# bghira/SimpleTuner

Hardware: NVIDIA H100
Metric: images/sec Flux.1-dev LoRA bf16 1024^2 (higher is better)
Workload: dtype bf16

## Files before the change

### simpletuner_b200/csrc/api.cu

```cuda
#include <cuda.h>
#include <cudaTypedefs.h>
#include <cuda_runtime.h>

#include <algorithm>
#include <atomic>
#include <cstdarg>
#include <cstdio>
#include <cmath>
#include <cstdlib>
#include <cstring>
#include <mutex>
#include <string>
#include <unordered_map>

#include <climits>
#include "../../include/stb200.h"
#include "attn_bwd.cuh"
#include "attn_fwd.cuh"
#include "optim.cuh"
#include "elementwise.cuh"
#include "gemm.cuh"
#include "lokr.cuh"
#include "vae.cuh"
#include "wgrad.cuh"
// ... 176 lines not shown
    cfg.attrs = attr;
    cfg.numAttrs = 1;
    static std::atomic<int> max_clusters{0};
    int mc = max_clusters.load(std::memory_order_acquire);
    if (mc == 0) {
      cfg.gridDim = dim3(CLUSTER * (num_sms() / CLUSTER));
      STB_CUDA(cudaOccupancyMaxActiveClusters(&mc, kernel, &cfg));
      if (mc < 1) return fail(STB_ERR_CUDA, "%s: no %d-CTA cluster of this kernel fits on the device", name, CLUSTER);
      max_clusters.store(mc, std::memory_order_release);
    }
    cfg.gridDim = dim3((unsigned)(CLUSTER * std::min<long long>(units, mc)));
    STB_CUDA(cudaLaunchKernelEx(&cfg, kernel, maps, p));
  }
  STB_LAUNCH_CHECK(name);
  return 0;
}

template <int BN>
int launch_gemm(const stb_gemm_args* a, cudaStream_t st, bool cluster) {
  stb::GemmMaps maps;
  std::memset(&maps, 0, sizeof maps);
  stb::GemmParams p;
  std::memset(&p, 0, sizeof p);
  for (int s = 0; s < a->nseg; ++s) {
    const stb_gemm_seg& g = a->seg[s];
    if (g.K <= 0 || (g.K & 7)) return fail(STB_ERR_ARG, "segment %d: K=%d must be a positive multiple of 8", s, g.K);
    if (int r = make_token_map(&maps.a[s], g.a, g.K, a->rows_per_batch, a->num_batches, g.a_row_stride, g.a_batch_stride,
                               stb::GemmCfg<BN>::BM))
      return r;
    if (g.w_kn) {
      unsigned long long wd[2] = {(unsigned long long)a->N, (unsigned long long)g.K};
      unsigned long long ws[1] = {(unsigned long long)g.w_row_stride * 2ull};
      unsigned wb[2] = {64, 64};
      if (int r = make_map(&maps.w[s], g.w, 2, wd, ws, wb)) return r;
    } else {
      unsigned long long wd[2] = {(unsigned long long)g.K, (unsigned long long)a->N};
      unsigned long long ws[1] = {(unsigned long long)g.w_row_stride * 2ull};
      unsigned wb[2] = {64, cluster ? 64u : (unsigned)BN};
      if (int r = make_map(&maps.w[s], g.w, 2, wd, ws, wb)) return r;
    }
    p.w_kn[s] = g.w_kn ? 1 : 0;
    p.kblocks[s] = (g.K + 63) / 64;
  }
  p.rows_per_batch = a->rows_per_batch;
  p.num_batches = a->num_batches;
  p.N = a->N;
  p.nseg = a->nseg;
  p.nan_to_num = a->nan_to_num;
  p.D = static_cast<__nv_bfloat16*>(a->d);
  p.d_batch_stride = a->d_batch_stride;
  p.d_row_stride = a->d_row_stride;
  p.bias = static_cast<const __nv_bfloat16*>(a->bias);
  p.gate = static_cast<const __nv_bfloat16*>(a->gate);
  p.gate_batch_stride = a->gate_batch_stride;
  p.res = static_cast<const __nv_bfloat16*>(a->res);
  p.res_batch_stride = a->res_batch_stride;
  p.res_row_stride = a->res_row_stride;
  p.aux = static_cast<__nv_bfloat16*>(a->aux);
  p.aux_batch_stride = a->aux_batch_stride;
  p.aux_row_stride = a->aux_row_stride;
  auto go = [&](auto epi) -> int {
    constexpr int EPI = decltype(epi)::value;
    if constexpr (BN == 128)
      if (cluster) return launch_gemm_kernel<BN, EPI, false, 2>(maps, p, st, "gemm_bf16_tn_cluster");
    return launch_gemm_kernel<BN, EPI, false>(maps, p, st, "gemm_bf16_tn");
  };
  switch (a->epi) {
    case stb::EPI_STORE: return go(std::integral_constant<int, stb::EPI_STORE>{});
    case stb::EPI_GELU: return go(std::integral_constant<int, stb::EPI_GELU>{});
    case stb::EPI_GATE_RES: return go(std::integral_constant<int, stb::EPI_GATE_RES>{});
    case stb::EPI_MUL_DGELU: return go(std::integral_constant<int, stb::EPI_MUL_DGELU>{});
    case stb::EPI_ADD_RES: return go(std::integral_constant<int, stb::EPI_ADD_RES>{});
    case stb::EPI_MUL: return go(std::integral_constant<int, stb::EPI_MUL>{});
    case stb::EPI_QUICK_GELU: return go(std::integral_constant<int, stb::EPI_QUICK_GELU>{});
  }
  return fail(STB_ERR_ARG, "unknown epilogue %d", a->epi);
}

bool aligned16(const void* p) { return (reinterpret_cast<uintptr_t>(p) & 15) == 0; }

}

template <int HD, bool BIAS, bool KEY = false>
static int launch_attn_fwd(const stb::AttnFwdMaps& maps, const stb::AttnFwdParams& p, dim3 grid, cudaStream_t st) {
  using Cfg = stb::AttnFwdCfg<HD>;
  constexpr int SMEM = Cfg::SMEM_BYTES + (KEY ? Cfg::KV_STAGES * 128 * 4 : 0);
  if (int r = set_smem<stb::attn_fwd_kernel<HD, BIAS, KEY>>(SMEM)) return r;
  stb::attn_fwd_kernel<HD, BIAS, KEY><<<grid, 384, SMEM, st>>>(maps, p);
  STB_LAUNCH_CHECK(KEY ? "attn_fwd_key_bias" : (BIAS ? "attn_fwd_bias" : "attn_fwd"));
  return 0;
}

template <int HD, bool BIAS>
static int launch_attn_bwd(const stb_attn_bwd_args* a, const stb::AttnBwdMaps& maps, const stb::AttnBwdParams& p,
                           cudaStream_t st) {
  {
    const long long warps = (long long)a->B * a->Sq * a->H;
    stb::attn_bwd_delta_kernel<HD><<<(unsigned)((warps + 7) / 8), 256, 0, st>>>(
        static_cast<const __nv_bfloat16*>(a->o), a->o_b, a->o_s, a->o_h,
        static_cast<const __nv_bfloat16*>(a->d_o), a->do_b, a->do_s, a->do_h, a->delta, a->B, a->H, a->Sq);
    STB_LAUNCH_CHECK("attn_bwd_delta");
  }
  using Cfg = stb::AttnBwdCfg<HD>;
  constexpr int SMEM1 = Cfg::DKDV_SMEM_BYTES, SMEM2 = Cfg::DQ_SMEM_BYTES + (BIAS ? Cfg::STAGES * Cfg::KB : 0);
  if (int r = set_smem<stb::attn_bwd_dkdv_kernel<HD, BIAS>>(SMEM1)) return r;
  if (int r = set_smem<stb::attn_bwd_dq_kernel<HD, BIAS>>(SMEM2)) return r;
  stb::attn_bwd_dkdv_kernel<HD, BIAS><<<dim3((a->Sk + 63) / 64, a->H, a->B), 384, SMEM1, st>>>(maps, p);
  STB_LAUNCH_CHECK(BIAS ? "attn_bwd_dkdv_bias" : "attn_bwd_dkdv");
  stb::attn_bwd_dq_kernel<HD, BIAS><<<dim3((a->Sq + 127) / 128, a->H, a->B), 384, SMEM2, st>>>(maps, p);
  STB_LAUNCH_CHECK(BIAS ? "attn_bwd_dq_bias" : "attn_bwd_dq");
  return 0;
}

template <int BN, int OUT>
static int launch_wgrad(const stb::WgradMaps& maps, stb::WgradParams p, cudaStream_t st) {
  constexpr int SMEM = stb::WgradCfg<BN, OUT>::SMEM_BYTES;
  if (int r = set_smem<stb::wgrad_kernel<BN, OUT>>(SMEM)) return r;
  p.col_tiles = (p.K + BN - 1) / BN;
  const int units = p.splits * ((p.N + 127) / 128) * p.col_tiles;
  const int grid = OUT == stb::WGRAD_OUT_BF16_NK ? std::min(units, num_sms()) : units;
  stb::wgrad_kernel<BN, OUT><<<grid, 384, SMEM, st>>>(maps, p);
  STB_LAUNCH_CHECK(OUT == stb::WGRAD_OUT_BF16_NK ? "wgrad_full" : "wgrad_tn");
  return 0;
}

extern "C" {

const char* stb_last_error(void) { return g_err.c_str(); }
int stb_version(void) { return 100; }
long long stb_launch_count(void) { return g_launches.load(); }
void stb_reset_launch_count(void) { g_launches.store(0); }

int stb_gemm_bf16(const stb_gemm_args* a, void* stream) {
  if (int r = check_device()) return r;
  if (!a || a->nseg < 1 || a->nseg > 3) return fail(STB_ERR_ARG, "nseg must be 1..3");
  if (a->num_batches < 1 || a->rows_per_batch < 1 || a->N < 1) return fail(STB_ERR_ARG, "empty problem");
  if (!aligned16(a->d) || (a->d_row_stride & 7) || (a->d_batch_stride & 7))
    return fail(STB_ERR_ARG, "D must be 16-byte aligned with strides multiple of 8 elements");
  if (a->bias && !aligned16(a->bias)) return fail(STB_ERR_ARG, "bias must be 16-byte aligned");
  if (a->epi == STB_EPI_GATE_RES && (!a->gate || !a->res)) return fail(STB_ERR_ARG, "GATE_RES needs gate and res");
  if (a->epi == STB_EPI_GATE_RES && (!aligned16(a->gate) || (a->gate_batch_stride & 7)))
    return fail(STB_ERR_ARG, "gate must be 16-byte aligned");
  if ((a->epi == STB_EPI_GATE_RES || a->epi == STB_EPI_ADD_RES) &&
      (!a->res || !aligned16(a->res) || (a->res_row_stride & 7) || (a->res_batch_stride & 7)))
    return fail(STB_ERR_ARG, "res must be given, 16-byte aligned, strides multiple of 8");
  if ((a->epi == STB_EPI_MUL_DGELU || a->epi == STB_EPI_MUL) && !a->aux) return fail(STB_ERR_ARG, "MUL_DGELU / MUL need aux");
  if (a->aux && (!aligned16(a->aux) || (a->aux_row_stride & 7) || (a->aux_batch_stride & 7)))
    return fail(STB_ERR_ARG, "aux must be 16-byte aligned, strides multiple of 8");
  if (a->epi < 0 || a->epi > 6) return fail(STB_ERR_ARG, "unknown epilogue %d", a->epi);
  cudaStream_t st = static_cast<cudaStream_t>(stream);
  if (a->tile_mt < 0 || a->tile_mt > 2) return fail(STB_ERR_ARG, "unsupported tile config MT=%d", a->tile_mt);
  int bn = a->tile_bn;
  if (bn == 0) {
    bn = a->N <= 64 ? 64 : (a->rows_per_batch <= 64 && a->N > 128 ? 256 : 128);
  }
  if (bn == 256) return launch_gemm<256>(a, st, false);
  if (bn == 128) {
    const long long tiles_m = (long long)((a->rows_per_batch + 127) / 128) * a->num_batches;
    const bool cluster = a->tile_mt == 2 || (a->tile_mt == 0 && tiles_m >= 16 &&
                                             (a->epi == STB_EPI_GELU || a->epi == STB_EPI_MUL_DGELU));
    return launch_gemm<128>(a, st, cluster);
  }
  if (bn == 64) return launch_gemm<64>(a, st, false);
  return fail(STB_ERR_ARG, "unsupported tile config BN=%d", bn);
}

int stb_attn_fwd(const stb_attn_fwd_args* a, void* stream) {
  if (int r = check_device()) return r;
  if (!a || a->B < 1 || a->H < 1 || a->Sq < 1 || a->Sk < 1) return fail(STB_ERR_ARG, "empty attention problem");
  if (a->HD != 128 && a->HD != 64) return fail(STB_ERR_UNSUPPORTED, "head_dim %d not supported (64 or 128)", a->HD);
  if (!aligned16(a->o) || (a->o_s & 7) || (a->o_h & 7) || (a->o_b & 7)) return fail(STB_ERR_ARG, "O alignment");
  cudaStream_t st = static_cast<cudaStream_t>(stream);
  stb::AttnFwdMaps maps;
  auto mk = [&](CUtensorMap* m, const void* ptr, long long sb, long long ss, long long sh, int S) {
    return make_head_map(m, ptr, a->HD, a->H, S, a->B, sb, ss, sh, 128);
  };
  if (int r = mk(&maps.q, a->q, a->q_b, a->q_s, a->q_h, a->Sq)) return r;
  if (int r = mk(&maps.k, a->k, a->k_b, a->k_s, a->k_h, a->Sk)) return r;
  if (int r = mk(&maps.v, a->v, a->v_b, a->v_s, a->v_h, a->Sk)) return r;
  stb::AttnFwdParams p;
  p.B = a->B; p.H = a->H; p.Sq = a->Sq; p.Sk = a->Sk;
  p.scale = a->scale;
  p.O = static_cast<__nv_bfloat16*>(a->o);
  p.o_b = a->o_b; p.o_s = a->o_s; p.o_h = a->o_h;
  p.lse = a->lse;
  p.bias = static_cast<const __nv_bfloat16*>(a->bias);
  p.bias_b = a->bias_b; p.bias_h = a->bias_h; p.bias_q = a->bias_q;
  p.inv_scale = a->scale != 0.f ? 1.f / a->scale : 0.f;
  const dim3 grid((a->Sq + 127) / 128, a->H, a->B);
  if (a->bias) {
    const bool key_row = a->bias_q == 0 && a->bias_h == 0;
    if (a->scale == 0.f || a->bias_b < 0 || a->bias_h < 0 || (a->bias_q < a->Sk && !key_row))
      return fail(STB_ERR_ARG, "attn_fwd bias: scale must be non-zero, strides non-negative, and bias_q >= Sk "
                               "(or bias_q = bias_h = 0 for a per-key row)");
    if (key_row)
      return a->HD == 128 ? launch_attn_fwd<128, true, true>(maps, p, grid, st) : launch_attn_fwd<64, true, true>(maps, p, grid, st);
    return a->HD == 128 ? launch_attn_fwd<128, true>(maps, p, grid, st) : launch_attn_fwd<64, true>(maps, p, grid, st);
  }
  return a->HD == 128 ? launch_attn_fwd<128, false>(maps, p, grid, st) : launch_attn_fwd<64, false>(maps, p, grid, st);
}

int stb_attn_bwd(const stb_attn_bwd_args* a, void* stream) {
  if (int r = check_device()) return r;
  if (!a || a->B < 1 || a->H < 1 || a->Sq < 1 || a->Sk < 1) return fail(STB_ERR_ARG, "empty attention problem");
  if (a->HD != 128 && a->HD != 64) return fail(STB_ERR_UNSUPPORTED, "head_dim %d not supported (64 or 128)", a->HD);
  if (!a->lse || !a->delta) return fail(STB_ERR_ARG, "attn_bwd needs lse and a delta scratch buffer");
  auto al = [&](const void* ptr, long long sb, long long ss, long long sh) {
    return aligned16(ptr) && !(sb & 7) && !(ss & 7) && !(sh & 7);
  };
  if (!al(a->dq, a->dq_b, a->dq_s, a->dq_h) || !al(a->dk, a->dk_b, a->dk_s, a->dk_h) ||
      !al(a->dv, a->dv_b, a->dv_s, a->dv_h))
    return fail(STB_ERR_ARG, "dq/dk/dv must be 16-byte aligned with strides multiple of 8 elements");
  cudaStream_t st = static_cast<cudaStream_t>(stream);
  stb::AttnBwdMaps maps;
  auto mk = [&](CUtensorMap* m, const void* ptr, long long sb, long long ss, long long sh, int S, unsigned rows) {
    return make_head_map(m, ptr, a->HD, a->H, S, a->B, sb, ss, sh, rows);
  };
  if (int r = mk(&maps.q128, a->q, a->q_b, a->q_s, a->q_h, a->Sq, 128)) return r;
  if (int r = mk(&maps.do128, a->d_o, a->do_b, a->do_s, a->do_h, a->Sq, 128)) return r;
  if (int r = mk(&maps.q64, a->q, a->q_b, a->q_s, a->q_h, a->Sq, 64)) return r;
  if (int r = mk(&maps.k64, a->k, a->k_b, a->k_s, a->k_h, a->Sk, 64)) return r;
  if (int r = mk(&maps.v64, a->v, a->v_b, a->v_s, a->v_h, a->Sk, 64)) return r;
  if (int r = mk(&maps.do64, a->d_o, a->do_b, a->do_s, a->do_h, a->Sq, 64)) return r;
  stb::AttnBwdParams p;
  p.B = a->B; p.H = a->H; p.Sq = a->Sq; p.Sk = a->Sk;
  p.scale = a->scale;
  p.lse = a->lse;
  p.delta = a->delta;
  p.dq = static_cast<__nv_bfloat16*>(a->dq);
  p.dk = static_cast<__nv_bfloat16*>(a->dk);
  p.dv = static_cast<__nv_bfloat16*>(a->dv);
  p.dq_b = a->dq_b; p.dq_s = a->dq_s; p.dq_h = a->dq_h;
  p.dk_b = a->dk_b; p.dk_s = a->dk_s; p.dk_h = a->dk_h;
  p.dv_b = a->dv_b; p.dv_s = a->dv_s; p.dv_h = a->dv_h;
  p.fuse_prep = 0;
  if (const stb_qk_prep* f = a->qk_prep) {
    if (a->Sq != a->Sk) return fail(STB_ERR_ARG, "qk_prep fusion needs self-attention (Sq == Sk)");
    if (!f->src || !aligned16(f->src) || (f->src_b & 7) || (f->src_s & 7) || (f->k_off & 7))
      return fail(STB_ERR_ARG, "qk_prep.src must be 16-byte aligned with strides / k_off multiple of 8 elements");
    if ((f->cos_t == nullptr) != (f->sin_t == nullptr)) return fail(STB_ERR_ARG, "qk_prep: give both cos_t and sin_t or neither");
    p.fuse_prep = 1;
    p.src = static_cast<const __nv_bfloat16*>(f->src);
    p.src_b = f->src_b; p.src_s = f->src_s; p.k_off = f->k_off;
    p.wq0 = static_cast<const __nv_bfloat16*>(f->wq); p.wk0 = static_cast<const __nv_bfloat16*>(f->wk);
    p.wq1 = static_cast<const __nv_bfloat16*>(f->wq_added); p.wk1 = static_cast<const __nv_bfloat16*>(f->wk_added);
    p.s_split = f->s_split;
    p.cosT = f->cos_t; p.sinT = f->sin_t;
    p.eps = f->eps;
  }
  p.q = static_cast<const __nv_bfloat16*>(a->q);
  p.d_o = static_cast<const __nv_bfloat16*>(a->d_o);
  p.q_b = a->q_b; p.q_s = a->q_s; p.q_h = a->q_h;
  p.do_b = a->do_b; p.do_s = a->do_s; p.do_h = a->do_h;
  p.bias = static_cast<const __nv_bfloat16*>(a->bias);
  p.bias_b = a->bias_b;
  if (a->bias) {
    if (a->bias_b < 0 || (a->bias_b != 0 && a->bias_b < a->Sk))
      return fail(STB_ERR_UNSUPPORTED, "attn_bwd bias: only a per-key bias [B or 1, Sk] (bias_b = 0 or >= Sk) is supported");
    return a->HD == 128 ? launch_attn_bwd<128, true>(a, maps, p, st) : launch_attn_bwd<64, true>(a, maps, p, st);
  }
  return a->HD == 128 ? launch_attn_bwd<128, false>(a, maps, p, st) : launch_attn_bwd<64, false>(a, maps, p, st);
}

int stb_ln_modulate_fwd(const void* x, long long x_b, long long x_s, const void* shift, const void* scale,
                        long long mod_b, void* out, long long o_b, long long o_s, int B, int S, int D,
                        float eps, void* stream) {
  if (int r = check_device()) return r;
  if ((D & 7) || D > 8192) return fail(STB_ERR_ARG, "D=%d must be a multiple of 8 and <= 8192", D);
  if (!aligned16(x) || !aligned16(out) || !aligned16(shift) || !aligned16(scale) || (x_s & 7) || (x_b & 7) ||
      (o_s & 7) || (o_b & 7) || (mod_b & 7))
    return fail(STB_ERR_ARG, "ln_modulate_fwd alignment");
  cudaStream_t st = static_cast<cudaStream_t>(stream);
  const int rows = B * S;
  const int vpt = (D + 1023) / 1024;
  auto X = static_cast<const __nv_bfloat16*>(x);
  auto SH = static_cast<const __nv_bfloat16*>(shift);
  auto SC = static_cast<const __nv_bfloat16*>(scale);
  auto O = static_cast<__nv_bfloat16*>(out);
#define STB_LN_F(V) stb::ln_modulate_fwd_kernel<V><<<rows, 128, 0, st>>>(X, x_b, x_s, SH, SC, mod_b, O, o_b, o_s, S, D, eps)
  switch (vpt) {
    case 1: STB_LN_F(1); break;
    case 2: STB_LN_F(2); break;
// ... 562 lines not shown
```

### simpletuner_b200/csrc/attn_bwd.cuh

```cuda
#pragma once
#include "../../include/stb200.h"
#include "attn_fwd.cuh"
#include "common.cuh"
#include "elementwise.cuh"

namespace stb {

struct AttnBwdParams {
  int B, H, Sq, Sk;
  float scale;
  const float* lse;
  const float* delta;
  __nv_bfloat16 *dq, *dk, *dv;
  long long dq_b, dq_s, dq_h, dk_b, dk_s, dk_h, dv_b, dv_s, dv_h;
  const __nv_bfloat16 *q, *d_o;
  long long q_b, q_s, q_h, do_b, do_s, do_h;
  int fuse_prep;
  const __nv_bfloat16* src;
  long long src_b, src_s;
  int k_off;
  const __nv_bfloat16 *wq0, *wk0, *wq1, *wk1;
  int s_split;
  const float *cosT, *sinT;
  float eps;
  const __nv_bfloat16* bias;
  long long bias_b;
};

struct AttnBwdMaps {
  CUtensorMap q128, do128, q64, k64, v64, do64;
};

template <int HD>
__global__ void __launch_bounds__(256)
attn_bwd_delta_kernel(const __nv_bfloat16* __restrict__ o, long long o_b, long long o_s, long long o_h,
                      const __nv_bfloat16* __restrict__ d_o, long long do_b, long long do_s, long long do_h,
                      float* __restrict__ delta, int B, int H, int S) {
  constexpr int EPL = HD / 32;
  const long long wid = (long long)blockIdx.x * 8 + (threadIdx.x >> 5);
  if (wid >= (long long)B * S * H) return;
  const int lane = threadIdx.x & 31;
  const int h = int(wid % H);
  const long long r = wid / H;
  const int s = int(r % S);
  const int b = int(r / S);
  const __nv_bfloat16* po = o + b * o_b + s * o_s + h * o_h + lane * EPL;
  const __nv_bfloat16* pg = d_o + b * do_b + s * do_s + h * do_h + lane * EPL;
  float acc = 0.f;
#pragma unroll
  for (int i = 0; i < EPL; ++i) acc += __bfloat162float(po[i]) * __bfloat162float(pg[i]);
#pragma unroll
  for (int off = 16; off > 0; off >>= 1) acc += __shfl_xor_sync(0xffffffffu, acc, off);
  if (lane == 0) delta[((long long)b * H + h) * S + s] = acc;
}

template <int HD>
struct AttnBwdCfg {
  static constexpr int BIG = 128 * HD * 2;
  static constexpr int SMALL = 64 * HD * 2;
  static constexpr int STAGES = 3;
  static constexpr int STAT = 64 * 8;
  static constexpr int PT = 64 * 64 * 4;
  static constexpr int DKDV_SMEM_BYTES = 2 * SMALL + STAGES * (2 * SMALL + STAT) + 2 * PT + 1024 + 256;
  static constexpr int DQ_SMEM_BYTES = 2 * BIG + STAGES * 2 * SMALL + 1024 + 256;
  static constexpr int KB = 64 * 4;
};

__device__ __forceinline__ void named_bar_sync(int id, int nthreads) {
  asm volatile("bar.sync %0, %1;" ::"r"(id), "r"(nthreads) : "memory");
}
__device__ __forceinline__ void named_bar_arrive(int id, int nthreads) {
  asm volatile("bar.arrive %0, %1;" ::"r"(id), "r"(nthreads) : "memory");
}

template <int HD>
__device__ __forceinline__ void stage_acc(float* rows, const float (&acc)[HD / 2], float mul) {
  const int t = threadIdx.x & 127, wq = t >> 5, lane = t & 31;
#pragma unroll
  for (int i = 0; i < HD / 8; ++i)
#pragma unroll
    for (int hh = 0; hh < 2; ++hh) {
      float* r = rows + (wq * 16 + (lane >> 2) + 8 * hh) * (HD + 4) + 8 * i + 2 * (lane & 3);
      r[0] = acc[4 * i + 2 * hh] * mul;
      r[1] = acc[4 * i + 2 * hh + 1] * mul;
    }
}

template <int HD>
__device__ __forceinline__ void store_row_half(const float* row, int half, __nv_bfloat16* grow, bool row_ok, bool prep,
                                               const __nv_bfloat16* xrow, const __nv_bfloat16* w, const float* cs,
                                               const float* sn, float eps) {
  constexpr int NC = HD / 2;
  const int c0 = half * NC;
  if (!prep) {
    if (row_ok) {
#pragma unroll
      for (int c = 0; c < NC; c += 8) {
        float o[8];
#pragma unroll
        for (int i = 0; i < 8; ++i) o[i] = row[c0 + c + i];
        *reinterpret_cast<uint4*>(grow + c0 + c) = pack8(o);
      }
    }
    return;
  }
  float ss = 0.f, sgx = 0.f;
  float g[NC];
#pragma unroll
  for (int c = 0; c < NC; c += 8) {
    float x[8], wv[8];
    unpack8(row_ok ? __ldg(reinterpret_cast<const uint4*>(xrow + c0 + c)) : make_uint4(0u, 0u, 0u, 0u), x);
    if (w) unpack8(__ldg(reinterpret_cast<const uint4*>(w + c0 + c)), wv);
#pragma unroll
    for (int i = 0; i < 8; i += 2) {
      const int j = c0 + c + i;
      const float go0 = row[j], go1 = row[j + 1];
      float dy0 = go0, dy1 = go1;
      if (cs && row_ok) {
        const float2 c2 = __ldg(reinterpret_cast<const float2*>(cs + j));
        const float2 s2 = __ldg(reinterpret_cast<const float2*>(sn + j));
        dy0 = go0 * c2.x + go1 * s2.y;
        dy1 = go1 * c2.y - go0 * s2.x;
      }
      const float g0 = w ? dy0 * wv[i] : dy0, g1 = w ? dy1 * wv[i + 1] : dy1;
      ss += x[i] * x[i] + x[i + 1] * x[i + 1];
      sgx += g0 * x[i] + g1 * x[i + 1];
      g[c + i] = g0;
      g[c + i + 1] = g1;
    }
  }
  ss += __shfl_xor_sync(0xffffffffu, ss, 1);
  sgx += __shfl_xor_sync(0xffffffffu, sgx, 1);
  const float rstd = rsqrtf(ss / HD + eps);
  const float m = sgx * rstd / HD;
  if (row_ok) {
#pragma unroll
    for (int c = 0; c < NC; c += 8) {
      float x[8], o[8];
      unpack8(__ldg(reinterpret_cast<const uint4*>(xrow + c0 + c)), x);
#pragma unroll
      for (int i = 0; i < 8; ++i) o[i] = rstd * (g[c + i] - (x[i] * rstd) * m);
      *reinterpret_cast<uint4*>(grow + c0 + c) = pack8(o);
    }
  }
}

__device__ __forceinline__ void wgmma_ss_n64_zero(float (&d)[32], uint64_t a, uint64_t b) {
  asm volatile(
      "{\n\t.reg .pred p;\n\tsetp.ne.b32 p, %34, 0;\n\t"
      "wgmma.mma_async.sync.aligned.m64n64k16.f32.bf16.bf16 {%0, %1, %2, %3, %4, %5, %6, %7, %8, %9, %10, %11, %12, %13, "
      "%14, %15, %16, %17, %18, %19, %20, %21, %22, %23, %24, %25, %26, %27, %28, %29, %30, %31}, %32, %33, p, 1, 1, 0, 0;\n\t}\n"
      : "=f"(d[0]), "=f"(d[1]), "=f"(d[2]), "=f"(d[3]), "=f"(d[4]), "=f"(d[5]), "=f"(d[6]), "=f"(d[7]), "=f"(d[8]),
        "=f"(d[9]), "=f"(d[10]), "=f"(d[11]), "=f"(d[12]), "=f"(d[13]), "=f"(d[14]), "=f"(d[15]), "=f"(d[16]),
        "=f"(d[17]), "=f"(d[18]), "=f"(d[19]), "=f"(d[20]), "=f"(d[21]), "=f"(d[22]), "=f"(d[23]), "=f"(d[24]),
        "=f"(d[25]), "=f"(d[26]), "=f"(d[27]), "=f"(d[28]), "=f"(d[29]), "=f"(d[30]), "=f"(d[31])
      : "l"(a), "l"(b), "r"(0u));
// ... 359 lines not shown
```

### simpletuner_b200/csrc/attn_fwd.cuh

```cuda
#pragma once
#include "common.cuh"

namespace stb {

struct AttnFwdParams {
  int B, H, Sq, Sk;
  float scale;
  __nv_bfloat16* O;
  long long o_b, o_s, o_h;
  float* lse;
  const __nv_bfloat16* bias;
  long long bias_h, bias_q;
  float inv_scale;
  long long bias_b;
};

struct AttnFwdMaps {
  CUtensorMap q, k, v;
};

template <int HD>
struct AttnFwdCfg {
  static constexpr int ATOMS = HD / 64;
  static constexpr int TILE_BYTES = 128 * HD * 2;
  static constexpr int KV_STAGES = 2;
  static constexpr int SMEM_BYTES = TILE_BYTES + KV_STAGES * 2 * TILE_BYTES + 1024 + 256;
  static constexpr int THREADS = 384;
};

template <int R>
__device__ __forceinline__ void acc_to_afrag(const float (&d)[R], int kk, uint32_t (&a)[4]) {
  a[0] = pack_bf16x2(d[8 * kk + 0], d[8 * kk + 1]);
  a[1] = pack_bf16x2(d[8 * kk + 2], d[8 * kk + 3]);
  a[2] = pack_bf16x2(d[8 * kk + 4], d[8 * kk + 5]);
  a[3] = pack_bf16x2(d[8 * kk + 6], d[8 * kk + 7]);
}

template <int N>
__device__ __forceinline__ void wgmma_rs_mn(float (&d)[N / 2], const uint32_t (&a)[4], uint64_t b, uint32_t accumulate) {
  if constexpr (N == 128) wgmma_rs_n128<1>(d, a, b, accumulate);
  else wgmma_rs_n64<1>(d, a, b, accumulate);
}

template <int HD, bool BIAS = false, bool KEY = false>
__global__ void __launch_bounds__(384, 1)
attn_fwd_kernel(const __grid_constant__ AttnFwdMaps maps, const AttnFwdParams p) {
  using Cfg = AttnFwdCfg<HD>;
  constexpr int ATOMS = Cfg::ATOMS;
  constexpr int TILE = Cfg::TILE_BYTES;
  constexpr int ATOM_BYTES = 128 * 64 * 2;
  constexpr int NSTG = Cfg::KV_STAGES;

  extern __shared__ uint8_t smem_raw[];
  const uint32_t smem_base = (smem_u32(smem_raw) + 1023u) & ~1023u;
  const uint32_t q_smem = smem_base;
  const uint32_t k_smem = q_smem + TILE;
  const uint32_t v_smem = k_smem + NSTG * TILE;
  const uint32_t bar_base = v_smem + NSTG * TILE;
  const uint32_t q_full = bar_base;
  auto k_full = [&](int s) { return bar_base + 8u * (1 + s); };
  auto k_empty = [&](int s) { return bar_base + 8u * (1 + NSTG + s); };
  auto v_full = [&](int s) { return bar_base + 8u * (1 + 2 * NSTG + s); };
  auto v_empty = [&](int s) { return bar_base + 8u * (1 + 3 * NSTG + s); };
  auto b_full = [&](int s) { return bar_base + 8u * (1 + 4 * NSTG + s); };
  auto b_empty = [&](int s) { return bar_base + 8u * (1 + 5 * NSTG + s); };
  float* kb_rows = reinterpret_cast<float*>(smem_raw + (bar_base + 256 - smem_u32(smem_raw)));

  const int warp = threadIdx.x >> 5;
  const int lane = threadIdx.x & 31;
  const int wg = __shfl_sync(0xffffffffu, warp >> 2, 0);
  const int q0 = blockIdx.x * 128;
  const int h = blockIdx.y;
  const int b = blockIdx.z;
  const int n_kv = (p.Sk + 127) / 128;

  if (threadIdx.x == 0) {
    tma_prefetch_desc(&maps.q);
    tma_prefetch_desc(&maps.k);
    tma_prefetch_desc(&maps.v);
    mbar_init(q_full, 1);
    for (int s = 0; s < NSTG; ++s) {
      mbar_init(k_full(s), 1);
      mbar_init(k_empty(s), 8);
      mbar_init(v_full(s), 1);
      mbar_init(v_empty(s), 8);
      if constexpr (KEY) {
        mbar_init(b_full(s), 1);
        mbar_init(b_empty(s), 8);
      }
    }
    fence_mbar_init();
  }
  __syncthreads();

  if (wg == 0) {
    reg_dealloc<40>();
    if (warp == 0) {
      if (elect_one()) {
        mbar_arrive_expect_tx(q_full, TILE);
        for (int a = 0; a < ATOMS; ++a) tma_load_4d(q_smem + a * ATOM_BYTES, &maps.q, q_full, a * 64, h, q0, b);
      }
      __syncwarp();
      for (int j = 0; j < n_kv; ++j) {
        const int stg = j % NSTG;
        const uint32_t par = ((j / NSTG) & 1) ^ 1u;
        mbar_wait(k_empty(stg), par, 10);
        if (elect_one()) {
          mbar_arrive_expect_tx(k_full(stg), TILE);
          for (int a = 0; a < ATOMS; ++a)
            tma_load_4d(k_smem + stg * TILE + a * ATOM_BYTES, &maps.k, k_full(stg), a * 64, h, j * 128, b);
        }
        __syncwarp();
        mbar_wait(v_empty(stg), par, 11);
        if (elect_one()) {
          mbar_arrive_expect_tx(v_full(stg), TILE);
          for (int a = 0; a < ATOMS; ++a)
            tma_load_4d(v_smem + stg * TILE + a * ATOM_BYTES, &maps.v, v_full(stg), a * 64, h, j * 128, b);
        }
        __syncwarp();
        if constexpr (KEY) {
          mbar_wait(b_empty(stg), par, 12);
          const __nv_bfloat16* brow = p.bias + (long long)b * p.bias_b + (long long)j * 128;
#pragma unroll
          for (int r = lane; r < 128; r += 32) kb_rows[stg * 128 + r] = j * 128 + r < p.Sk ? __bfloat162float(brow[r]) : 0.f;
          __syncwarp();
          if (lane == 0) mbar_arrive(b_full(stg));
        }
      }
    }
  } else {
    reg_alloc<232>();
    const int cw = wg - 1;
    const int wq = warp & 3;
    const int r_lo = q0 + cw * 64 + wq * 16 + (lane >> 2);
    const float sl2 = p.scale * 1.4426950408889634f;
    float s_acc[64];
    float o_acc[HD / 2];
#pragma unroll
    for (int i = 0; i < HD / 2; ++i) o_acc[i] = 0.f;
    float m_row[2] = {-INFINITY, -INFINITY};
    float l_row[2] = {0.f, 0.f};
    const __nv_bfloat16* brow[2] = {nullptr, nullptr};
    if constexpr (BIAS && !KEY) {
#pragma unroll
      for (int hh = 0; hh < 2; ++hh)
        brow[hh] = p.bias + (long long)b * p.bias_b + (long long)h * p.bias_h +
                   (long long)min(r_lo + 8 * hh, p.Sq - 1) * p.bias_q;
    }
    const uint32_t qa = q_smem + cw * 8192;
    mbar_wait(q_full, 0, 20);

    for (int j = 0; j < n_kv; ++j) {
      const int stg = j % NSTG;
      const uint32_t par = (j / NSTG) & 1;
      mbar_wait(k_full(stg), par, 21);
      const uint32_t ka = k_smem + stg * TILE;
      wg_fence();
#pragma unroll
      for (int kk = 0; kk < HD / 16; ++kk) {
        const uint32_t off = (kk / 4) * ATOM_BYTES + (kk % 4) * 32;
        wgmma_ss_n128<0, 0>(s_acc, sdesc_k(qa, off), sdesc_k(ka, off), kk > 0 ? 1u : 0u);
      }
      wg_commit();
      wg_wait<0>();
      wg_fence_regs(s_acc);
      __syncwarp();
      if (lane == 0) mbar_arrive(k_empty(stg));

      const int kv_valid = p.Sk - j * 128;
      if constexpr (KEY) mbar_wait(b_full(stg), par, 23);
#pragma unroll
      for (int i = 0; i < 16; ++i) {
        float2 kb2 = make_float2(0.f, 0.f);
        if constexpr (KEY) kb2 = reinterpret_cast<const float2*>(kb_rows + stg * 128)[4 * i + (lane & 3)];
#pragma unroll
        for (int e = 0; e < 2; ++e) {
          const int c = 8 * i + 2 * (lane & 3) + e;
#pragma unroll
          for (int hh = 0; hh < 2; ++hh) {
            float v = s_acc[4 * i + 2 * hh + e];
            if constexpr (KEY) {
              if (c < kv_valid) v = fmaf(e ? kb2.y : kb2.x, p.inv_scale, v);
            } else if constexpr (BIAS) {
              if (c < kv_valid) v = fmaf(__bfloat162float(brow[hh][j * 128 + c]), p.inv_scale, v);
            }
            if (c >= kv_valid) v = -INFINITY;
            s_acc[4 * i + 2 * hh + e] = v;
          }
        }
      }
      if constexpr (KEY) {
        __syncwarp();
        if (lane == 0) mbar_arrive(b_empty(stg));
      }
      float alpha[2], nmb[2];
#pragma unroll
      for (int hh = 0; hh < 2; ++hh) {
        float m = -INFINITY;
#pragma unroll
        for (int i = 0; i < 16; ++i) m = fmaxf(m, fmaxf(s_acc[4 * i + 2 * hh], s_acc[4 * i + 2 * hh + 1]));
        m = fmaxf(m, __shfl_xor_sync(0xffffffffu, m, 1));
        m = fmaxf(m, __shfl_xor_sync(0xffffffffu, m, 2));
        const float m_new = fmaxf(m_row[hh], m);
        const float m_exp = (BIAS && m_new == -INFINITY) ? 0.f : m_new;
        alpha[hh] = ex2f((m_row[hh] - m_exp) * sl2);
        m_row[hh] = m_new;
        nmb[hh] = -m_exp * sl2;
        l_row[hh] *= alpha[hh];
      }
#pragma unroll
      for (int i = 0; i < HD / 8; ++i) {
        o_acc[4 * i + 0] *= alpha[0];
        o_acc[4 * i + 1] *= alpha[0];
        o_acc[4 * i + 2] *= alpha[1];
        o_acc[4 * i + 3] *= alpha[1];
      }
#pragma unroll
      for (int i = 0; i < 16; ++i) {
#pragma unroll
        for (int hh = 0; hh < 2; ++hh) {
#pragma unroll
          for (int e = 0; e < 2; ++e) {
            const float x = ex2f(fmaf(s_acc[4 * i + 2 * hh + e], sl2, nmb[hh]));
            l_row[hh] += x;
            s_acc[4 * i + 2 * hh + e] = x;
          }
        }
      }

      mbar_wait(v_full(stg), par, 22);
      const uint32_t va = v_smem + stg * TILE;
      wg_fence();
#pragma unroll
      for (int kk = 0; kk < 8; ++kk) {
        uint32_t a[4];
        acc_to_afrag(s_acc, kk, a);
        wgmma_rs_mn<HD>(o_acc, a, sdesc_mn(va, kk * 2048, ATOM_BYTES), 1u);
      }
      wg_commit();
      wg_wait<0>();
      wg_fence_regs(o_acc);
      __syncwarp();
      if (lane == 0) mbar_arrive(v_empty(stg));
    }

#pragma unroll
    for (int hh = 0; hh < 2; ++hh) {
      float l = l_row[hh];
      l += __shfl_xor_sync(0xffffffffu, l, 1);
      l += __shfl_xor_sync(0xffffffffu, l, 2);
      const int s = r_lo + 8 * hh;
      const float inv_l = 1.f / l;
      if (s < p.Sq) {
        __nv_bfloat16* orow = p.O + (long long)b * p.o_b + (long long)s * p.o_s + (long long)h * p.o_h;
#pragma unroll
        for (int i = 0; i < HD / 8; ++i)
          *reinterpret_cast<uint32_t*>(orow + 8 * i + 2 * (lane & 3)) =
              pack_bf16x2(o_acc[4 * i + 2 * hh] * inv_l, o_acc[4 * i + 2 * hh + 1] * inv_l);
        if (p.lse && (lane & 3) == 0) p.lse[((long long)b * p.H + h) * p.Sq + s] = m_row[hh] * p.scale + logf(l);
      }
    }
  }
}

}
```

Before: 1.963.

## Make attention forward persistent with deeper KV pipeline and ping-pong overlap

Converts the forward attention kernel into a persistent kernel that loops over (q-tile, head, batch) units with a grid capped at the SM count. A q_empty barrier lets the producer reload Q for the next unit. KV stages go from 2 to 3. For head_dim 64 it adds intra-warpgroup overlap (the PV matmul of the previous tile is issued alongside the next QK matmul) and named-barrier ping-pong between the two consumer warpgroups. This aims to hide launch tails and the MMA/softmax serialization, but it adds shared memory use and more complex barrier parity logic.

Result: no change. 1.966 (median of 6 runs) (+0.2%).

```diff
diff --git a/simpletuner_b200/csrc/api.cu b/simpletuner_b200/csrc/api.cu
--- a/simpletuner_b200/csrc/api.cu
+++ b/simpletuner_b200/csrc/api.cu
@@ -282,10 +282,12 @@
 }
 
 template <int HD, bool BIAS, bool KEY = false>
-static int launch_attn_fwd(const stb::AttnFwdMaps& maps, const stb::AttnFwdParams& p, dim3 grid, cudaStream_t st) {
+static int launch_attn_fwd(const stb::AttnFwdMaps& maps, const stb::AttnFwdParams& p, cudaStream_t st) {
   using Cfg = stb::AttnFwdCfg<HD>;
   constexpr int SMEM = Cfg::SMEM_BYTES + (KEY ? Cfg::KV_STAGES * 128 * 4 : 0);
   if (int r = set_smem<stb::attn_fwd_kernel<HD, BIAS, KEY>>(SMEM)) return r;
+  const long long units = (long long)((p.Sq + 127) / 128) * p.H * p.B;
+  const int grid = (int)std::min<long long>(units, num_sms());
   stb::attn_fwd_kernel<HD, BIAS, KEY><<<grid, 384, SMEM, st>>>(maps, p);
   STB_LAUNCH_CHECK(KEY ? "attn_fwd_key_bias" : (BIAS ? "attn_fwd_bias" : "attn_fwd"));
   return 0;
@@ -387,17 +389,16 @@
   p.bias = static_cast<const __nv_bfloat16*>(a->bias);
   p.bias_b = a->bias_b; p.bias_h = a->bias_h; p.bias_q = a->bias_q;
   p.inv_scale = a->scale != 0.f ? 1.f / a->scale : 0.f;
-  const dim3 grid((a->Sq + 127) / 128, a->H, a->B);
   if (a->bias) {
     const bool key_row = a->bias_q == 0 && a->bias_h == 0;
     if (a->scale == 0.f || a->bias_b < 0 || a->bias_h < 0 || (a->bias_q < a->Sk && !key_row))
       return fail(STB_ERR_ARG, "attn_fwd bias: scale must be non-zero, strides non-negative, and bias_q >= Sk "
                                "(or bias_q = bias_h = 0 for a per-key row)");
     if (key_row)
-      return a->HD == 128 ? launch_attn_fwd<128, true, true>(maps, p, grid, st) : launch_attn_fwd<64, true, true>(maps, p, grid, st);
-    return a->HD == 128 ? launch_attn_fwd<128, true>(maps, p, grid, st) : launch_attn_fwd<64, true>(maps, p, grid, st);
-  }
-  return a->HD == 128 ? launch_attn_fwd<128, false>(maps, p, grid, st) : launch_attn_fwd<64, false>(maps, p, grid, st);
+      return a->HD == 128 ? launch_attn_fwd<128, true, true>(maps, p, st) : launch_attn_fwd<64, true, true>(maps, p, st);
+    return a->HD == 128 ? launch_attn_fwd<128, true>(maps, p, st) : launch_attn_fwd<64, true>(maps, p, st);
+  }
+  return a->HD == 128 ? launch_attn_fwd<128, false>(maps, p, st) : launch_attn_fwd<64, false>(maps, p, st);
 }
 
 int stb_attn_bwd(const stb_attn_bwd_args* a, void* stream) {
diff --git a/simpletuner_b200/csrc/attn_bwd.cuh b/simpletuner_b200/csrc/attn_bwd.cuh
--- a/simpletuner_b200/csrc/attn_bwd.cuh
+++ b/simpletuner_b200/csrc/attn_bwd.cuh
@@ -65,13 +65,6 @@
   static constexpr int DQ_SMEM_BYTES = 2 * BIG + STAGES * 2 * SMALL + 1024 + 256;
   static constexpr int KB = 64 * 4;
 };
-
-__device__ __forceinline__ void named_bar_sync(int id, int nthreads) {
-  asm volatile("bar.sync %0, %1;" ::"r"(id), "r"(nthreads) : "memory");
-}
-__device__ __forceinline__ void named_bar_arrive(int id, int nthreads) {
-  asm volatile("bar.arrive %0, %1;" ::"r"(id), "r"(nthreads) : "memory");
-}
 
 template <int HD>
 __device__ __forceinline__ void stage_acc(float* rows, const float (&acc)[HD / 2], float mul) {
diff --git a/simpletuner_b200/csrc/attn_fwd.cuh b/simpletuner_b200/csrc/attn_fwd.cuh
--- a/simpletuner_b200/csrc/attn_fwd.cuh
+++ b/simpletuner_b200/csrc/attn_fwd.cuh
@@ -23,7 +23,7 @@
 struct AttnFwdCfg {
   static constexpr int ATOMS = HD / 64;
   static constexpr int TILE_BYTES = 128 * HD * 2;
-  static constexpr int KV_STAGES = 2;
+  static constexpr int KV_STAGES = 3;
   static constexpr int SMEM_BYTES = TILE_BYTES + KV_STAGES * 2 * TILE_BYTES + 1024 + 256;
   static constexpr int THREADS = 384;
 };
@@ -40,6 +40,13 @@
 __device__ __forceinline__ void wgmma_rs_mn(float (&d)[N / 2], const uint32_t (&a)[4], uint64_t b, uint32_t accumulate) {
   if constexpr (N == 128) wgmma_rs_n128<1>(d, a, b, accumulate);
   else wgmma_rs_n64<1>(d, a, b, accumulate);
+}
+
+__device__ __forceinline__ void named_bar_sync(int id, int nthreads) {
+  asm volatile("bar.sync %0, %1;" ::"r"(id), "r"(nthreads) : "memory");
+}
+__device__ __forceinline__ void named_bar_arrive(int id, int nthreads) {
+  asm volatile("bar.arrive %0, %1;" ::"r"(id), "r"(nthreads) : "memory");
 }
 
 template <int HD, bool BIAS = false, bool KEY = false>
@@ -50,6 +57,8 @@
   constexpr int TILE = Cfg::TILE_BYTES;
   constexpr int ATOM_BYTES = 128 * 64 * 2;
   constexpr int NSTG = Cfg::KV_STAGES;
+  constexpr int TURN = 1;
+  constexpr bool OVERLAP = HD == 64;
 
   extern __shared__ uint8_t smem_raw[];
   const uint32_t smem_base = (smem_u32(smem_raw) + 1023u) & ~1023u;
@@ -58,6 +67,7 @@
   const uint32_t v_smem = k_smem + NSTG * TILE;
   const uint32_t bar_base = v_smem + NSTG * TILE;
   const uint32_t q_full = bar_base;
+  const uint32_t q_empty = bar_base + 8u * (1 + 6 * NSTG);
   auto k_full = [&](int s) { return bar_base + 8u * (1 + s); };
   auto k_empty = [&](int s) { return bar_base + 8u * (1 + NSTG + s); };
   auto v_full = [&](int s) { return bar_base + 8u * (1 + 2 * NSTG + s); };
@@ -69,9 +79,8 @@
   const int warp = threadIdx.x >> 5;
   const int lane = threadIdx.x & 31;
   const int wg = __shfl_sync(0xffffffffu, warp >> 2, 0);
-  const int q0 = blockIdx.x * 128;
-  const int h = blockIdx.y;
-  const int b = blockIdx.z;
+  const int n_qt = (p.Sq + 127) / 128;
+  const int units = n_qt * p.H * p.B;
   const int n_kv = (p.Sk + 127) / 128;
 
   if (threadIdx.x == 0) {
@@ -79,6 +88,7 @@
     tma_prefetch_desc(&maps.k);
     tma_prefetch_desc(&maps.v);
     mbar_init(q_full, 1);
+    mbar_init(q_empty, 8);
     for (int s = 0; s < NSTG; ++s) {
       mbar_init(k_full(s), 1);
       mbar_init(k_empty(s), 8);
@@ -96,35 +106,40 @@
   if (wg == 0) {
     reg_dealloc<40>();
     if (warp == 0) {
-      if (elect_one()) {
-        mbar_arrive_expect_tx(q_full, TILE);
-        for (int a = 0; a < ATOMS; ++a) tma_load_4d(q_smem + a * ATOM_BYTES, &maps.q, q_full, a * 64, h, q0, b);
-      }
-      __syncwarp();
-      for (int j = 0; j < n_kv; ++j) {
-        const int stg = j % NSTG;
-        const uint32_t par = ((j / NSTG) & 1) ^ 1u;
-        mbar_wait(k_empty(stg), par, 10);
+      int it = 0;
+      for (int u = blockIdx.x, n = 0; u < units; u += gridDim.x, ++n) {
+        const int q0 = (u % n_qt) * 128, h = (u / n_qt) % p.H, b = u / (n_qt * p.H);
+        mbar_wait(q_empty, (n & 1) ^ 1u, 13);
         if (elect_one()) {
-          mbar_arrive_expect_tx(k_full(stg), TILE);
-          for (int a = 0; a < ATOMS; ++a)
-            tma_load_4d(k_smem + stg * TILE + a * ATOM_BYTES, &maps.k, k_full(stg), a * 64, h, j * 128, b);
+          mbar_arrive_expect_tx(q_full, TILE);
+          for (int a = 0; a < ATOMS; ++a) tma_load_4d(q_smem + a * ATOM_BYTES, &maps.q, q_full, a * 64, h, q0, b);
         }
         __syncwarp();
-        mbar_wait(v_empty(stg), par, 11);
-        if (elect_one()) {
-          mbar_arrive_expect_tx(v_full(stg), TILE);
-          for (int a = 0; a < ATOMS; ++a)
-            tma_load_4d(v_smem + stg * TILE + a * ATOM_BYTES, &maps.v, v_full(stg), a * 64, h, j * 128, b);
-        }
-        __syncwarp();
-        if constexpr (KEY) {
-          mbar_wait(b_empty(stg), par, 12);
-          const __nv_bfloat16* brow = p.bias + (long long)b * p.bias_b + (long long)j * 128;
-#pragma unroll
-          for (int r = lane; r < 128; r += 32) kb_rows[stg * 128 + r] = j * 128 + r < p.Sk ? __bfloat162float(brow[r]) : 0.f;
+        for (int j = 0; j < n_kv; ++j, ++it) {
+          const int stg = it % NSTG;
+          const uint32_t par = ((it / NSTG) & 1) ^ 1u;
+          mbar_wait(k_empty(stg), par, 10);
+          if (elect_one()) {
+            mbar_arrive_expect_tx(k_full(stg), TILE);
+            for (int a = 0; a < ATOMS; ++a)
+              tma_load_4d(k_smem + stg * TILE + a * ATOM_BYTES, &maps.k, k_full(stg), a * 64, h, j * 128, b);
+          }
           __syncwarp();
-          if (lane == 0) mbar_arrive(b_full(stg));
+          mbar_wait(v_empty(stg), par, 11);
+          if (elect_one()) {
+            mbar_arrive_expect_tx(v_full(stg), TILE);
+            for (int a = 0; a < ATOMS; ++a)
+              tma_load_4d(v_smem + stg * TILE + a * ATOM_BYTES, &maps.v, v_full(stg), a * 64, h, j * 128, b);
+          }
+          __syncwarp();
+          if constexpr (KEY) {
+            mbar_wait(b_empty(stg), par, 12);
+            const __nv_bfloat16* brow = p.bias + (long long)b * p.bias_b + (long long)j * 128;
+#pragma unroll
+            for (int r = lane; r < 128; r += 32) kb_rows[stg * 128 + r] = j * 128 + r < p.Sk ? __bfloat162float(brow[r]) : 0.f;
+            __syncwarp();
+            if (lane == 0) mbar_arrive(b_full(stg));
+          }
         }
       }
     }
@@ -132,134 +147,183 @@
     reg_alloc<232>();
     const int cw = wg - 1;
     const int wq = warp & 3;
-    const int r_lo = q0 + cw * 64 + wq * 16 + (lane >> 2);
     const float sl2 = p.scale * 1.4426950408889634f;
-    float s_acc[64];
-    float o_acc[HD / 2];
-#pragma unroll
-    for (int i = 0; i < HD / 2; ++i) o_acc[i] = 0.f;
-    float m_row[2] = {-INFINITY, -INFINITY};
-    float l_row[2] = {0.f, 0.f};
-    const __nv_bfloat16* brow[2] = {nullptr, nullptr};
-    if constexpr (BIAS && !KEY) {
-#pragma unroll
-      for (int hh = 0; hh < 2; ++hh)
-        brow[hh] = p.bias + (long long)b * p.bias_b + (long long)h * p.bias_h +
-                   (long long)min(r_lo + 8 * hh, p.Sq - 1) * p.bias_q;
+    const uint32_t qa = q_smem + cw * 8192;
+    if (OVERLAP && cw == 1) named_bar_arrive(TURN, 256);
+    int it = 0;
+    for (int u = blockIdx.x, n = 0; u < units; u += gridDim.x, ++n) {
+      const int q0 = (u % n_qt) * 128, h = (u / n_qt) % p.H, b = u / (n_qt * p.H);
+      const int r_lo = q0 + cw * 64 + wq * 16 + (lane >> 2);
+      float s_acc[64];
+      uint32_t pf[OVERLAP ? 8 : 1][4];
+      float o_acc[HD / 2];
+#pragma unroll
+      for (int i = 0; i < HD / 2; ++i) o_acc[i] = 0.f;
+      float m_row[2] = {-INFINITY, -INFINITY};
+      float l_row[2] = {0.f, 0.f};
+      const __nv_bfloat16* brow[2] = {nullptr, nullptr};
+      if constexpr (BIAS && !KEY) {
+#pragma unroll
+        for (int hh = 0; hh < 2; ++hh)
+          brow[hh] = p.bias + (long long)b * p.bias_b + (long long)h * p.bias_h +
+                     (long long)min(r_lo + 8 * hh, p.Sq - 1) * p.bias_q;
+      }
+      mbar_wait(q_full, n & 1, 20);
+
+      for (int j = 0; j < n_kv; ++j) {
+        const int stg = (it + j) % NSTG, pstg = (it + j + NSTG - 1) % NSTG;
+        const uint32_t par = ((it + j) / NSTG) & 1;
+        mbar_wait(k_full(stg), par, 21);
+        if (OVERLAP && j > 0) mbar_wait(v_full(pstg), ((it + j - 1) / NSTG) & 1, 22);
+        if (OVERLAP) named_bar_sync(TURN + cw, 256);
+        const uint32_t ka = k_smem + stg * TILE;
+        wg_fence();
+#pragma unroll
+        for (int kk = 0; kk < HD / 16; ++kk) {
+          const uint32_t off = (kk / 4) * ATOM_BYTES + (kk % 4) * 32;
+          wgmma_ss_n128<0, 0>(s_acc, sdesc_k(qa, off), sdesc_k(ka, off), kk > 0 ? 1u : 0u);
+        }
+        wg_commit();
+        if constexpr (OVERLAP) {
+          if (j > 0) {
+            const uint32_t va = v_smem + pstg * TILE;
+#pragma unroll
+            for (int kk = 0; kk < 8; ++kk)
+              wgmma_rs_mn<HD>(o_acc, pf[kk], sdesc_mn(va, kk * 2048, ATOM_BYTES), 1u);
+          }
+          wg_commit();
+          named_bar_arrive(TURN + 1 - cw, 256);
+        }
+        wg_wait<OVERLAP ? 1 : 0>();
+        wg_fence_regs(s_acc);
+        __syncwarp();
+        if (lane == 0) {
+          mbar_arrive(k_empty(stg));
+          if (j == n_kv - 1) mbar_arrive(q_empty);
+        }
+        const int kv_valid = p.Sk - j * 128;
+        if constexpr (KEY) mbar_wait(b_full(stg), par, 23);
+#pragma unroll
+        for (int i = 0; i < 16; ++i) {
+          float2 kb2 = make_float2(0.f, 0.f);
+          if constexpr (KEY) kb2 = reinterpret_cast<const float2*>(kb_rows + stg * 128)[4 * i + (lane & 3)];
+#pragma unroll
+          for (int e = 0; e < 2; ++e) {
+            const int c = 8 * i + 2 * (lane & 3) + e;
+#pragma unroll
+            for (int hh = 0; hh < 2; ++hh) {
+              float v = s_acc[4 * i + 2 * hh + e];
+              if constexpr (KEY) {
+                if (c < kv_valid) v = fmaf(e ? kb2.y : kb2.x, p.inv_scale, v);
+              } else if constexpr (BIAS) {
+                if (c < kv_valid) v = fmaf(__bfloat162float(brow[hh][j * 128 + c]), p.inv_scale, v);
+              }
+              if (c >= kv_valid) v = -INFINITY;
+              s_acc[4 * i + 2 * hh + e] = v;
+            }
+          }
+        }
+        if constexpr (KEY) {
+          __syncwarp();
+          if (lane == 0) mbar_arrive(b_empty(stg));
+        }
+        float alpha[2], nmb[2];
+#pragma unroll
+        for (int hh = 0; hh < 2; ++hh) {
+          float m = -INFINITY;
+#pragma unroll
+          for (int i = 0; i < 16; ++i) m = fmaxf(m, fmaxf(s_acc[4 * i + 2 * hh], s_acc[4 * i + 2 * hh + 1]));
+          m = fmaxf(m, __shfl_xor_sync(0xffffffffu, m, 1));
+          m = fmaxf(m, __shfl_xor_sync(0xffffffffu, m, 2));
+          const float m_new = fmaxf(m_row[hh], m);
+          const float m_exp = (BIAS && m_new == -INFINITY) ? 0.f : m_new;
+          alpha[hh] = ex2f((m_row[hh] - m_exp) * sl2);
+          m_row[hh] = m_new;
+          nmb[hh] = -m_exp * sl2;
+          l_row[hh] *= alpha[hh];
+        }
+#pragma unroll
+        for (int i = 0; i < 16; ++i) {
+#pragma unroll
+          for (int hh = 0; hh < 2; ++hh) {
+#pragma unroll
+            for (int e = 0; e < 2; ++e) {
+              const float x = ex2f(fmaf(s_acc[4 * i + 2 * hh + e], sl2, nmb[hh]));
+              l_row[hh] += x;
+              s_acc[4 * i + 2 * hh + e] = x;
+            }
+          }
+        }
+        if constexpr (OVERLAP) {
+          wg_wait<0>();
+          wg_fence_regs(o_acc);
+          if (j > 0) {
+            __syncwarp();
+            if (lane == 0) mbar_arrive(v_empty(pstg));
+          }
+        }
+#pragma unroll
+        for (int i = 0; i < HD / 8; ++i) {
+          o_acc[4 * i + 0] *= alpha[0];
+          o_acc[4 * i + 1] *= alpha[0];
+          o_acc[4 * i + 2] *= alpha[1];
+          o_acc[4 * i + 3] *= alpha[1];
+        }
+        if constexpr (OVERLAP) {
+#pragma unroll
+          for (int kk = 0; kk < 8; ++kk) acc_to_afrag(s_acc, kk, pf[kk]);
+        } else {
+          mbar_wait(v_full(stg), par, 22);
+          const uint32_t va = v_smem + stg * TILE;
+          wg_fence();
+#pragma unroll
+          for (int kk = 0; kk < 8; ++kk) {
+            uint32_t a[4];
+            acc_to_afrag(s_acc, kk, a);
+            wgmma_rs_mn<HD>(o_acc, a, sdesc_mn(va, kk * 2048, ATOM_BYTES), 1u);
+          }
+          wg_commit();
+          wg_wait<0>();
+          wg_fence_regs(o_acc);
+          __syncwarp();
+          if (lane == 0) mbar_arrive(v_empty(stg));
+        }
+      }
+      if constexpr (OVERLAP) {
+        const int lstg = (it + n_kv - 1) % NSTG;
+        mbar_wait(v_full(lstg), ((it + n_kv - 1) / NSTG) & 1, 24);
+        named_bar_sync(TURN + cw, 256);
+        const uint32_t va = v_smem + lstg * TILE;
+        wg_fence();
+#pragma unroll
+        for (int kk = 0; kk < 8; ++kk) wgmma_rs_mn<HD>(o_acc, pf[kk], sdesc_mn(va, kk * 2048, ATOM_BYTES), 1u);
+        wg_commit();
+        named_bar_arrive(TURN + 1 - cw, 256);
+        wg_wait<0>();
+        wg_fence_regs(o_acc);
+        __syncwarp();
+        if (lane == 0) mbar_arrive(v_empty(lstg));
+      }
+      it += n_kv;
+
+#pragma unroll
+      for (int hh = 0; hh < 2; ++hh) {
+        float l = l_row[hh];
+        l += __shfl_xor_sync(0xffffffffu, l, 1);
+        l += __shfl_xor_sync(0xffffffffu, l, 2);
+        const int s = r_lo + 8 * hh;
+        const float inv_l = 1.f / l;
+        if (s < p.Sq) {
+          __nv_bfloat16* orow = p.O + (long long)b * p.o_b + (long long)s * p.o_s + (long long)h * p.o_h;
+#pragma unroll
+          for (int i = 0; i < HD / 8; ++i)
+            *reinterpret_cast<uint32_t*>(orow + 8 * i + 2 * (lane & 3)) =
+                pack_bf16x2(o_acc[4 * i + 2 * hh] * inv_l, o_acc[4 * i + 2 * hh + 1] * inv_l);
+          if (p.lse && (lane & 3) == 0) p.lse[((long long)b * p.H + h) * p.Sq + s] = m_row[hh] * p.scale + logf(l);
+        }
+      }
     }
-    const uint32_t qa = q_smem + cw * 8192;
-    mbar_wait(q_full, 0, 20);
-
-    for (int j = 0; j < n_kv; ++j) {
-      const int stg = j % NSTG;
-      const uint32_t par = (j / NSTG) & 1;
-      mbar_wait(k_full(stg), par, 21);
-      const uint32_t ka = k_smem + stg * TILE;
-      wg_fence();
-#pragma unroll
-      for (int kk = 0; kk < HD / 16; ++kk) {
-        const uint32_t off = (kk / 4) * ATOM_BYTES + (kk % 4) * 32;
-        wgmma_ss_n128<0, 0>(s_acc, sdesc_k(qa, off), sdesc_k(ka, off), kk > 0 ? 1u : 0u);
-      }
-      wg_commit();
-      wg_wait<0>();
-      wg_fence_regs(s_acc);
-      __syncwarp();
-      if (lane == 0) mbar_arrive(k_empty(stg));
-
-      const int kv_valid = p.Sk - j * 128;
-      if constexpr (KEY) mbar_wait(b_full(stg), par, 23);
-#pragma unroll
-      for (int i = 0; i < 16; ++i) {
-        float2 kb2 = make_float2(0.f, 0.f);
-        if constexpr (KEY) kb2 = reinterpret_cast<const float2*>(kb_rows + stg * 128)[4 * i + (lane & 3)];
-#pragma unroll
-        for (int e = 0; e < 2; ++e) {
-          const int c = 8 * i + 2 * (lane & 3) + e;
-#pragma unroll
-          for (int hh = 0; hh < 2; ++hh) {
-            float v = s_acc[4 * i + 2 * hh + e];
-            if constexpr (KEY) {
-              if (c < kv_valid) v = fmaf(e ? kb2.y : kb2.x, p.inv_scale, v);
-            } else if constexpr (BIAS) {
-              if (c < kv_valid) v = fmaf(__bfloat162float(brow[hh][j * 128 + c]), p.inv_scale, v);
-            }
-            if (c >= kv_valid) v = -INFINITY;
-            s_acc[4 * i + 2 * hh + e] = v;
-          }
-        }
-      }
-      if constexpr (KEY) {
-        __syncwarp();
-        if (lane == 0) mbar_arrive(b_empty(stg));
-      }
-      float alpha[2], nmb[2];
-#pragma unroll
-      for (int hh = 0; hh < 2; ++hh) {
-        float m = -INFINITY;
-#pragma unroll
-        for (int i = 0; i < 16; ++i) m = fmaxf(m, fmaxf(s_acc[4 * i + 2 * hh], s_acc[4 * i + 2 * hh + 1]));
-        m = fmaxf(m, __shfl_xor_sync(0xffffffffu, m, 1));
-        m = fmaxf(m, __shfl_xor_sync(0xffffffffu, m, 2));
-        const float m_new = fmaxf(m_row[hh], m);
-        const float m_exp = (BIAS && m_new == -INFINITY) ? 0.f : m_new;
-        alpha[hh] = ex2f((m_row[hh] - m_exp) * sl2);
-        m_row[hh] = m_new;
-        nmb[hh] = -m_exp * sl2;
-        l_row[hh] *= alpha[hh];
-      }
-#pragma unroll
-      for (int i = 0; i < HD / 8; ++i) {
-        o_acc[4 * i + 0] *= alpha[0];
-        o_acc[4 * i + 1] *= alpha[0];
-        o_acc[4 * i + 2] *= alpha[1];
-        o_acc[4 * i + 3] *= alpha[1];
-      }
-#pragma unroll
-      for (int i = 0; i < 16; ++i) {
-#pragma unroll
-        for (int hh = 0; hh < 2; ++hh) {
-#pragma unroll
-          for (int e = 0; e < 2; ++e) {
-            const float x = ex2f(fmaf(s_acc[4 * i + 2 * hh + e], sl2, nmb[hh]));
-            l_row[hh] += x;
-            s_acc[4 * i + 2 * hh + e] = x;
-          }
-        }
-      }
-
-      mbar_wait(v_full(stg), par, 22);
-      const uint32_t va = v_smem + stg * TILE;
-      wg_fence();
-#pragma unroll
-      for (int kk = 0; kk < 8; ++kk) {
-        uint32_t a[4];
-        acc_to_afrag(s_acc, kk, a);
-        wgmma_rs_mn<HD>(o_acc, a, sdesc_mn(va, kk * 2048, ATOM_BYTES), 1u);
-      }
-      wg_commit();
-      wg_wait<0>();
-      wg_fence_regs(o_acc);
-      __syncwarp();
-      if (lane == 0) mbar_arrive(v_empty(stg));
-    }
-
-#pragma unroll
-    for (int hh = 0; hh < 2; ++hh) {
-      float l = l_row[hh];
-      l += __shfl_xor_sync(0xffffffffu, l, 1);
-      l += __shfl_xor_sync(0xffffffffu, l, 2);
-      const int s = r_lo + 8 * hh;
-      const float inv_l = 1.f / l;
-      if (s < p.Sq) {
-        __nv_bfloat16* orow = p.O + (long long)b * p.o_b + (long long)s * p.o_s + (long long)h * p.o_h;
-#pragma unroll
-        for (int i = 0; i < HD / 8; ++i)
-          *reinterpret_cast<uint32_t*>(orow + 8 * i + 2 * (lane & 3)) =
-              pack_bf16x2(o_acc[4 * i + 2 * hh] * inv_l, o_acc[4 * i + 2 * hh + 1] * inv_l);
-        if (p.lse && (lane & 3) == 0) p.lse[((long long)b * p.H + h) * p.Sq + s] = m_row[hh] * p.scale + logf(l);
-      }
-    }
+    if (OVERLAP && cw == 0) named_bar_sync(TURN, 256);
   }
 }
 
```
